# jdalcorso/radar-sounder-crw

Hardware: AMD Instinct MI355X
Metric: radargram columns/sec (CRW fwd+bwd) (higher is better)
Workload: dtype f32 (conv2-5 multiply on the bf16 matrix cores with hi/lo operand pairs, fp32 accumulate: fp32-grade; everything else fp32); 1 GPU; one synthetic 512x4096 radargram per GPU per step = 8 items [T=32,N=63,16x16] (patch 16x16, overlap (8, 0)), tau=0.01, CNN encoder, fwd+bwd+all-reduce+Adam; parallelism=dp1 (independent sequences), chain=fp32 MFMA 16x16x4, prefix form, encoder_convs=bf16x3

## Files before the change

### radar-sounder-crw_amd/csrc/encoder_front.hip

```cpp
#include "crw_common.h"
#include <type_traits>
#include <cstdlib>

namespace crw {
namespace {

typedef __bf16 bf8 __attribute__((ext_vector_type(8)));
typedef short s4v __attribute__((ext_vector_type(4)));
typedef short s8v __attribute__((ext_vector_type(8)));
typedef __attribute__((address_space(3))) char *lds_cp;

__device__ inline uint16_t f2bf(float x) { return __builtin_bit_cast(uint16_t, (__bf16)x); }
__device__ inline float bf2f(uint16_t h) { return __builtin_bit_cast(float, (uint32_t)h << 16); }

__device__ inline void lds_barrier() { asm volatile("s_waitcnt lgkmcnt(0)\n\ts_barrier" ::: "memory"); }

constexpr int XPW = 18;
constexpr int C1W = 14, C1N = C1W * C1W;
constexpr int A1W = 13, A1PW = 15;
constexpr int C2W = 11, C2N = C2W * C2W;
constexpr int OW = 10, ON = 100;
constexpr int D2PW = 19;
constexpr int D2HALF = D2PW * D2PW * 32;
constexpr int KS2 = 7;
// ... 271 lines not shown
    for (int e = tid; e < ON * 32; e += NT) {
      const int c = e & 31, q = e >> 5, y = q / OW, x = q % OW;
      if (oy0 + y < Ho && ox0 + x < Wo) {
        const float *s2 = L.c2r + (y * C2W + x) * 32 + c;
        const float v = fmaxf(fmaxf(s2[0], s2[32]), fmaxf(s2[C2W * 32], s2[C2W * 32 + 32]));
        const uint16_t h = f2bf(v);
        const long o = (((long)pt * Ho + oy0 + y) * Wo + ox0 + x) * 32 + c;
        a.f.yh[o] = h;
        if (SPLIT == 3) a.f.yl[o] = f2bf(v - bf2f(h));
      }
    }
  }
}

__global__ __launch_bounds__(256) void pack_w2_kernel(const float *__restrict__ w, uint16_t *fh, uint16_t *fl,
                                                      uint16_t *bh, uint16_t *bl) {
  for (int e = blockIdx.x * 256 + threadIdx.x; e < KS2 * 32 * 32; e += gridDim.x * 256) {
    const int k = e & 31, co = (e >> 5) & 31, s = e >> 10;
    const int tap = 4 * s + (k >> 3), ci = k & 7;
    const float v = tap < 25 ? w[(co * 8 + ci) * 25 + tap] : 0.f;
    const uint16_t h = f2bf(v);
    fh[e] = h;
    if (fl) fl[e] = f2bf(v - bf2f(h));
  }
  for (int e = blockIdx.x * 256 + threadIdx.x; e < 25 * 8 * 32; e += gridDim.x * 256) {
    const int co = e & 31, ci = (e >> 5) & 7, tap = e >> 8;
    const float v = w[(co * 8 + ci) * 25 + tap];
    const uint16_t h = f2bf(v);
    bh[e] = h;
    if (bl) bl[e] = f2bf(v - bf2f(h));
  }
}

struct FrontBwdArgs {
  FrontArgs f;
  const uint16_t *w2bh, *w2bl;
  const float *dy;
  float *part;
  int patches_per_block;
  long long *stamps;
  int H, W, tiles_x, tiles_y;
};
[[maybe_unused]] constexpr int NPHASE = 10;
#ifdef CRW_CONV_STAMPS
#define FRONT_STAMP(k)                                                       \
  if (a.stamps && tid == 0) {                                                \
    const long long now_ = (long long)__builtin_amdgcn_s_memtime();          \
    phase_[k] += now_ - prev_;                                               \
    prev_ = now_;                                                            \
  }
#else
#define FRONT_STAMP(k)
#endif

__device__ inline s4v tr_read0(uint32_t lds_addr) {
  s4v v;
  asm volatile("ds_read_b64_tr_b16 %0, %1" : "=v"(v) : "v"(lds_addr) : "memory");
  return v;
}
__device__ inline bf8 tr_pair(uint32_t a_lo, uint32_t a_hi) {
  const s4v lo = tr_read0(a_lo), hi = tr_read0(a_hi);
  const s8v v = {lo[0], lo[1], lo[2], lo[3], hi[0], hi[1], hi[2], hi[3]};
  return __builtin_bit_cast(bf8, v);
}

__device__ inline int argmax4(float a, float b, float c, float d) {
  int k = 0;
  float m = a;
  if (b > m) { m = b; k = 1; }
  if (c > m) { m = c; k = 2; }
  if (d > m) { m = d; k = 3; }
  return k;
}

template <int W, int CS>
__device__ inline float pool_bwd_pixel(const float *__restrict__ in, const float *__restrict__ dout, int y, int x, int c) {
  const float *ctr = in + ((y + 1) * (W + 2) + x + 1) * CS + c;
  float nb[3][3], dv[2][2];
#pragma unroll
  for (int dy = 0; dy < 3; ++dy)
#pragma unroll
    for (int dx = 0; dx < 3; ++dx) nb[dy][dx] = ctr[((dy - 1) * (W + 2) + (dx - 1)) * CS];
#pragma unroll
  for (int dyw = 0; dyw < 2; ++dyw)
#pragma unroll
    for (int dxw = 0; dxw < 2; ++dxw) {
      const int wy = min(max(y - dyw, 0), W - 2), wx = min(max(x - dxw, 0), W - 2);
      dv[dyw][dxw] = dout[(wy * (W - 1) + wx) * CS + c];
    }
  const float mine = nb[1][1];
  float gsum = 0.f;
#pragma unroll
  for (int dyw = 0; dyw < 2; ++dyw)
#pragma unroll
    for (int dxw = 0; dxw < 2; ++dxw) {
      const int wy = y - dyw, wx = x - dxw;
      bool win = mine > 0.f && wy >= 0 && wy < W - 1 && wx >= 0 && wx < W - 1;
      const int k = dyw * 2 + dxw;
#pragma unroll
      for (int j = 0; j < 4; ++j)
        if (j != k) {
          const float v = nb[1 - dyw + (j >> 1)][1 - dxw + (j & 1)];
          win = win && (j < k ? mine > v : mine >= v);
        }
      gsum += win ? dv[dyw][dxw] : 0.f;
    }
// ... 459 lines not shown
#pragma unroll
          for (int tx = 0; tx < 5; ++tx) {
            float s1 = 0.f;
#pragma unroll
            for (int x = 0; x < TCW / 2; ++x) s1 = fmaf(dv[x], xv[x + tx], s1);
            dw1[tx] += s1;
          }
        }
      }
    }
    lds_barrier();
  }

  const int PART = 32 * 8 * 25 + 32 + 8 * cin * 25 + 8;
  float *out = a.part + (long)blockIdx.x * PART;
#pragma unroll
  for (int uu = 0; uu < 2; ++uu) {
    const int tl = wave + NWV * uu;
    const int tap = 2 * (tl >> 1) + (r16 >> 3);
    if (tl < 26 && tap < 25)
#pragma unroll
      for (int r = 0; r < 4; ++r) out[((16 * (tl & 1) + 4 * g + r) * 8 + (r16 & 7)) * 25 + tap] = wacc[uu][r];
  }
  __syncthreads();
  float *red = reinterpret_cast<float *>(lds);
  red[tid] = db2;
  __syncthreads();
  if (tid < 32) {
    float s = 0.f;
    for (int k = 0; k < NTH / 32; ++k) s += red[tid + 32 * k];
    out[32 * 8 * 25 + tid] = s;
  }
  __syncthreads();
  if (tid < nrowthr)
#pragma unroll
    for (int tx = 0; tx < 5; ++tx) red[tid * 5 + tx] = dw1[tx];
  __syncthreads();
  if (tid < nout) {
    const int q = tid / 5, tx = tid % 5;
    float s = 0.f;
    for (int y = 0; y < nrp; ++y) s += red[(q * nrp + y) * 5 + tx];
    out[32 * 8 * 25 + 32 + tid] = s;
  }
  __syncthreads();
  red[tid] = db1;
  __syncthreads();
  if (tid < 8) {
    float s = 0.f;
    for (int k = 0; k < NTH / 8; ++k) s += red[tid + 8 * k];
    out[32 * 8 * 25 + 32 + nout + tid] = s;
  }
}

template <int SPLIT>
__global__ __launch_bounds__(NTH) void front_bwd_saved_kernel(FrontBwdArgs a) {
  extern __shared__ __attribute__((aligned(16))) char lds[];
  char *p = lds;
  const int cin = a.f.cin;
  auto take = [&](size_t bytes) { char *r = p; p += (bytes + 15) & ~(size_t)15; return r; };
  float *xs = (float *)take(sizeof(float) * cin * XPW * XPW);
  char *a1h = take(A1PW * A1PW * 16), *a1l = take(A1PW * A1PW * 16);
  char *wbh = take(25 * 8 * 32 * 2), *wbl = take(25 * 8 * 32 * 2);
  char *d2h = take(2 * D2HALF), *d2l = take(2 * D2HALF);
  float *dyb = (float *)take(sizeof(float) * ON * 32);
  char *k2s = take(SV_K2), *k1s = take(SV_K1);
  float *dA1 = dyb, *dC1 = dyb + A1W * A1W * 8;

  const int tid = threadIdx.x, lane = tid & 63, wave = tid >> 6, g = lane >> 4, r16 = lane & 15;
  for (int e = tid; e < cin * XPW * XPW; e += NTH) xs[e] = 0.f;
  for (int e = tid; e < A1PW * A1PW * 4; e += NTH) {
    reinterpret_cast<uint32_t *>(a1h)[e] = 0;
    reinterpret_cast<uint32_t *>(a1l)[e] = 0;
  }
  for (int e = tid; e < 25 * 8 * 32 / 8; e += NTH) {
    const int ch = e & 3, ci = (e >> 2) & 7, tap = e >> 5;
    const int d = ((tap * 2 + (ch >> 1)) * 8 + ci) * 2 + (ch & 1);
    reinterpret_cast<uint4 *>(wbh)[d] = reinterpret_cast<const uint4 *>(a.w2bh)[e];
    if (SPLIT == 3) reinterpret_cast<uint4 *>(wbl)[d] = reinterpret_cast<const uint4 *>(a.w2bl)[e];
  }
  for (int e = tid; e < 2 * D2HALF / 4; e += NTH) {
    reinterpret_cast<uint32_t *>(d2h)[e] = 0;
    reinterpret_cast<uint32_t *>(d2l)[e] = 0;
  }
  __syncthreads();

  f32x4 wacc[2];
  wacc[0] = f32x4{0.f, 0.f, 0.f, 0.f};
  wacc[1] = f32x4{0.f, 0.f, 0.f, 0.f};
  float db2 = 0.f, db1 = 0.f, dw1[5] = {0.f, 0.f, 0.f, 0.f, 0.f};
  const int nout = 8 * cin * 25, nrp = C1W / cin, nrowthr = 8 * cin * 5 * nrp;
  const uint32_t d2h_a = (uint32_t)(uintptr_t)(lds_cp)d2h, d2l_a = (uint32_t)(uintptr_t)(lds_cp)d2l;
  const uint32_t a1h_a = (uint32_t)(uintptr_t)(lds_cp)a1h, a1l_a = (uint32_t)(uintptr_t)(lds_cp)a1l;
  const int p_begin = blockIdx.x * a.patches_per_block;
  const int p_end = min(a.f.P, p_begin + a.patches_per_block);

  constexpr int NA1 = 2 * SV_A1 / 16, NK2 = SV_K2 / 16, NK1 = SV_K1 / 16, NSV = NA1 + NK2 + NK1;
  static_assert(NSV <= NTH && ON * 32 / 4 <= NTH, "one chunk per thread");
  typedef uint32_t u4v __attribute__((ext_vector_type(4)));
  float4 dy_r;
  float x_r = 0.f;
  u4v sv_r;
  const __amdgpu_buffer_rsrc_t dy_rs = __builtin_amdgcn_make_buffer_rsrc((void *)a.dy, 0, (int)((long)a.f.P * ON * 32 * 4), 0x00020000);
  const __amdgpu_buffer_rsrc_t x_rs = __builtin_amdgcn_make_buffer_rsrc((void *)a.f.x, 0, (int)((long)a.f.P * cin * 256 * 4), 0x00020000);
  const __amdgpu_buffer_rsrc_t sv_rs = __builtin_amdgcn_make_buffer_rsrc((void *)a.f.saved, 0, (int)((long)a.f.P * SV_BYTES), 0x00020000);
  auto fetch = [&](int pt) {
    dy_r = __builtin_bit_cast(float4, __builtin_amdgcn_raw_buffer_load_b128(dy_rs, tid * 16, pt * (ON * 32 * 4), 0));
    x_r = __builtin_bit_cast(float, __builtin_amdgcn_raw_buffer_load_b32(x_rs, tid * 4, pt * (cin * 256 * 4), 0));
    sv_r = __builtin_amdgcn_raw_buffer_load_b128(sv_rs, min(tid, NSV - 1) * 16, pt * SV_BYTES, 0);
  };
  if (p_begin < p_end) fetch(p_begin);
  for (int pt = p_begin; pt < p_end; ++pt) {
    if (tid < cin * 256) xs[((tid >> 8) * XPW + ((tid >> 4) & 15) + 1) * XPW + (tid & 15) + 1] = x_r;
    if (tid < ON * 32 / 4) reinterpret_cast<float4 *>(dyb)[tid] = dy_r;
    if (tid < NA1) {
      const int pl = tid / (A1W * A1W), px = tid % (A1W * A1W);
      *reinterpret_cast<u4v *>((pl ? a1l : a1h) + ((px / A1W + 1) * A1PW + px % A1W + 1) * 16) = sv_r;
    } else if (tid < NA1 + NK2) {
      reinterpret_cast<u4v *>(k2s)[tid - NA1] = sv_r;
    } else if (tid < NSV) {
      reinterpret_cast<u4v *>(k1s)[tid - NA1 - NK2] = sv_r;
    }
    if (pt + 1 < p_end) fetch(pt + 1);
    lds_barrier();

    for (int e = tid; e < C2N * 32; e += NTH) {
      const int co = e & 31, pix = e >> 5, y = pix / C2W, x = pix % C2W;
      float gsum = 0.f;
#pragma unroll
      for (int dyw = 0; dyw < 2; ++dyw)
#pragma unroll
        for (int dxw = 0; dxw < 2; ++dxw) {
          const int wy = y - dyw, wx = x - dxw;
          const bool ok = wy >= 0 && wy < OW && wx >= 0 && wx < OW;
          const int idx = (min(max(wy, 0), OW - 1) * OW + min(max(wx, 0), OW - 1)) * 32 + co;
          const int code = k2s[idx];
          const float d = dyb[idx];
          gsum += (ok && code == (4 | (dyw * 2 + dxw))) ? d : 0.f;
        }
      db2 += gsum;
      const uint16_t h = f2bf(gsum);
      const int o = (co >> 4) * D2HALF + ((y + 4) * D2PW + x + 4) * 32 + 2 * (co & 15);
      *reinterpret_cast<uint16_t *>(d2h + o) = h;
      if (SPLIT == 3) *reinterpret_cast<uint16_t *>(d2l + o) = f2bf(gsum - bf2f(h));
    }
    lds_barrier();

    {
      const int t16 = lane & 15, q = t16 >> 2, pq = t16 & 3;
#pragma unroll 1
      for (int ks = 0; ks < 4; ++ks) {
        const int i_lo = 32 * ks + 8 * g + q, i_hi = i_lo + 4;
        const bool v_lo = i_lo < C2N, v_hi = i_hi < C2N;
        const int y_lo = v_lo ? i_lo / C2W : 0, x_lo = v_lo ? i_lo % C2W : 0;
        const int y_hi = v_hi ? i_hi / C2W : 0, x_hi = v_hi ? i_hi % C2W : 0;
        const uint32_t ya_lo = (v_lo ? ((y_lo + 4) * D2PW + x_lo + 4) : 0) * 32 + 8 * (pq & 1) + 16 * (pq >> 1);
        const uint32_t ya_hi = (v_hi ? ((y_hi + 4) * D2PW + x_hi + 4) : 0) * 32 + 8 * (pq & 1) + 16 * (pq >> 1);
#pragma unroll
        for (int u = 0; u < 2; ++u) {
          const int tile = wave + NWV * u;
          if (tile < 26) {
            const int i = tile & 1, nt = tile >> 1;
            int tap = 2 * nt + (pq >> 1);
            if (tap > 24) tap = 24;
            const int toff = (tap / 5) * A1PW + (tap % 5);
            const uint32_t xa_lo = ((y_lo * A1PW + x_lo) + toff) * 16 + 8 * (pq & 1);
            const uint32_t xa_hi = ((y_hi * A1PW + x_hi) + toff) * 16 + 8 * (pq & 1);
            const bf8 ah = tr_pair(d2h_a + ya_lo + D2HALF * i, d2h_a + ya_hi + D2HALF * i);
            const bf8 bh = tr_pair(a1h_a + xa_lo, a1h_a + xa_hi);
            bf8 al, bl;
            if (SPLIT == 3) {
              al = tr_pair(d2l_a + ya_lo + D2HALF * i, d2l_a + ya_hi + D2HALF * i);
              bl = tr_pair(a1l_a + xa_lo, a1l_a + xa_hi);
            }
            asm volatile("s_waitcnt lgkmcnt(0)" ::: "memory");
            __builtin_amdgcn_sched_barrier(0);
            if (SPLIT == 3) {
              wacc[u] = __builtin_amdgcn_mfma_f32_16x16x32_bf16(al, bh, wacc[u], 0, 0, 0);
              wacc[u] = __builtin_amdgcn_mfma_f32_16x16x32_bf16(ah, bl, wacc[u], 0, 0, 0);
            }
            wacc[u] = __builtin_amdgcn_mfma_f32_16x16x32_bf16(ah, bh, wacc[u], 0, 0, 0);
          }
        }
      }
    }
    {
      f32x4 dacc = f32x4{0.f, 0.f, 0.f, 0.f}, dacc1 = dacc;
      if (wave < A1W) {
        const int xl = (r16 >= 4 && r16 < 12) ? r16 - 4 : (r16 < 4 ? 8 + r16 : 12);
        const int base = (wave + 5) * D2PW + xl + 5;
        const char *wb = ((SPLIT == 3 && r16 >= 8) ? wbl : wbh) + (g >> 1) * 256 + (r16 & 7) * 32 + (g & 1) * 16;
        const char *ab = d2h + (g >> 1) * D2HALF + (base - (4 * D2PW + 4)) * 32 + (g & 1) * 16;
        const long lo_a = d2l - d2h;
#pragma unroll
        for (int tap = 0; tap < 25; ++tap) {
          const int arel = ((4 - tap / 5) * D2PW + (4 - tap % 5)) * 32;
          const bf8 b = *reinterpret_cast<const bf8 *>(wb + tap * 512);
          const bf8 ah = *reinterpret_cast<const bf8 *>(ab + arel);
          if (SPLIT == 3) {
            const bf8 al = *reinterpret_cast<const bf8 *>(ab + lo_a + arel);
            dacc1 = __builtin_amdgcn_mfma_f32_16x16x32_bf16(al, b, dacc1, 0, 0, 0);
          }
          dacc = __builtin_amdgcn_mfma_f32_16x16x32_bf16(ah, b, dacc, 0, 0, 0);
        }
        if (SPLIT == 3) {
#pragma unroll
          for (int r = 0; r < 4; ++r) dacc[r] += __shfl_down(dacc[r], 8, 64) + dacc1[r];
        }
      }
      lds_barrier();
      if (wave < A1W && r16 < 8)
#pragma unroll
        for (int r = 0; r < 4; ++r) {
          const int row = 4 * g + r;
          const int x = (row >= 4 && row < 12) ? row - 4 : (row < 4 ? 8 + row : 12);
          if (row < 13) dA1[(wave * A1W + x) * 8 + r16] = dacc[r];
        }
    }
    lds_barrier();

    for (int e = tid; e < C1N * 8; e += NTH) {
      const int co = e & 7, pix = e >> 3, y = pix / C1W, x = pix % C1W;
      float gsum = 0.f;
#pragma unroll
      for (int dyw = 0; dyw < 2; ++dyw)
#pragma unroll
        for (int dxw = 0; dxw < 2; ++dxw) {
          const int wy = y - dyw, wx = x - dxw;
          const bool ok = wy >= 0 && wy < A1W && wx >= 0 && wx < A1W;
          const int idx = (min(max(wy, 0), A1W - 1) * A1W + min(max(wx, 0), A1W - 1)) * 8 + co;
          const int code = k1s[idx];
          const float d = dA1[idx];
          gsum += (ok && code == (4 | (dyw * 2 + dxw))) ? d : 0.f;
        }
      dC1[co * C1N + pix] = gsum;
      db1 += gsum;
    }
    lds_barrier();

    if (tid < nrowthr) {
      const int rp = tid % nrp, q = tid / nrp, ty = q % 5, ci = (q / 5) % cin, co = q / (5 * cin);
      for (int y = rp; y < C1W; y += nrp) {
        const float *dr = dC1 + co * C1N + y * C1W, *xr = xs + (ci * XPW + y + ty) * XPW;
        float dv[C1W], xv[XPW];
#pragma unroll
        for (int x = 0; x < C1W; ++x) dv[x] = dr[x];
#pragma unroll
        for (int x = 0; x < XPW; ++x) xv[x] = xr[x];
#pragma unroll
        for (int tx = 0; tx < 5; ++tx) {
          float s1 = 0.f;
#pragma unroll
          for (int x = 0; x < C1W; ++x) s1 = fmaf(dv[x], xv[x + tx], s1);
          dw1[tx] += s1;
        }
      }
    }
    lds_barrier();
  }

  const int PART = 32 * 8 * 25 + 32 + 8 * cin * 25 + 8;
  float *out = a.part + (long)blockIdx.x * PART;
#pragma unroll
  for (int u = 0; u < 2; ++u) {
    const int tile = wave + NWV * u;
    const int tap = 2 * (tile >> 1) + (r16 >> 3);
    if (tile < 26 && tap < 25)
#pragma unroll
      for (int r = 0; r < 4; ++r) out[((16 * (tile & 1) + 4 * g + r) * 8 + (r16 & 7)) * 25 + tap] = wacc[u][r];
  }
  __syncthreads();
  float *red = reinterpret_cast<float *>(lds);
  red[tid] = db2;
  __syncthreads();
  if (tid < 32) {
    float s = 0.f;
    for (int k = 0; k < NTH / 32; ++k) s += red[tid + 32 * k];
    out[32 * 8 * 25 + tid] = s;
  }
  __syncthreads();
  if (tid < nrowthr)
#pragma unroll
    for (int tx = 0; tx < 5; ++tx) red[tid * 5 + tx] = dw1[tx];
  __syncthreads();
  if (tid < nout) {
    const int q = tid / 5, tx = tid % 5;
    float s = 0.f;
    for (int y = 0; y < nrp; ++y) s += red[(q * nrp + y) * 5 + tx];
    out[32 * 8 * 25 + 32 + tid] = s;
  }
  __syncthreads();
  red[tid] = db1;
  __syncthreads();
  if (tid < 8) {
    float s = 0.f;
    for (int k = 0; k < NTH / 8; ++k) s += red[tid + 8 * k];
    out[32 * 8 * 25 + 32 + nout + tid] = s;
  }
}

struct FrontSums {
  const float *part;
  int nslice, stride, n;
  int end[4];
  float *dst[4];
};
__global__ __launch_bounds__(256) void front_slice_sum_kernel(FrontSums a) {
  const int e = blockIdx.x * 4 + (threadIdx.x >> 6), lane = threadIdx.x & 63;
  if (e >= a.n) return;
  float s = 0.f;
  for (int k = lane; k < a.nslice; k += 64) s += a.part[(long)k * a.stride + e];
  s = wave_sum(s);
  if (lane == 0) {
    const int seg = e < a.end[0] ? 0 : e < a.end[1] ? 1 : e < a.end[2] ? 2 : 3;
    a.dst[seg][e - (seg ? a.end[seg - 1] : 0)] = s;
  }
}

size_t fwd_lds_bytes(int cin, bool pad = false) {
  auto r = [](size_t b) { return (b + 15) & ~(size_t)15; };
  const size_t c1 = pad ? (C1W + 2) * (C1W + 2) : C1N, c2 = pad ? (C2W + 2) * (C2W + 2) : C2N;
  return r(4 * cin * XPW * XPW) + r(4 * (8 * cin * 25 + 8)) + r(4 * c1 * 8) + 2 * r(A1PW * A1PW * 16) +
         2 * r(KS2 * 32 * 32 * 2) + r(4 * c2 * 32);
}
size_t bwd_lds_bytes(int cin) {
  auto r = [](size_t b) { return (b + 15) & ~(size_t)15; };
  return fwd_lds_bytes(cin, true) + 2 * r(25 * 8 * 32 * 2) + 2 * r(2 * D2HALF) + r(4 * ON * 32);
}
size_t bwd_saved_lds_bytes(int cin) {
  auto r = [](size_t b) { return (b + 15) & ~(size_t)15; };
  return r(4 * cin * XPW * XPW) + 2 * r(A1PW * A1PW * 16) + 2 * r(25 * 8 * 32 * 2) + 2 * r(2 * D2HALF) + r(4 * ON * 32) + r(SV_K2) + r(SV_K1);
}
int front_slices(int P) { return P < 256 ? P : 256; }

}
}

using namespace crw;

long long *g_front_stamps = nullptr;

extern "C" {

#ifdef CRW_CONV_STAMPS
void crw_debug_front_stamps(long long *buf) { g_front_stamps = buf; }
#endif

int crw_enc_front_pack(const float *w2, uint16_t *fwd_hi, uint16_t *fwd_lo, uint16_t *bwd_hi, uint16_t *bwd_lo,
                       crw_stream_t stream) {
  clear_stale_error();
  if (!w2 || !fwd_hi || !bwd_hi || (fwd_lo == nullptr) != (bwd_lo == nullptr)) return CRW_EINVAL;
  hipLaunchKernelGGL(pack_w2_kernel, dim3(28), dim3(256), 0, (hipStream_t)stream, w2, fwd_hi, fwd_lo, bwd_hi, bwd_lo);
  return check_launch();
}

static int front_fwd_threads() {
  static const int nt = [] { const char *e = getenv("CRW_FRONT_NT"); return e && atoi(e) == 1024 ? 1024 : 512; }();
  return nt;
}

size_t crw_enc_front_saved_bytes(int P) { return P < 1 ? 0 : (size_t)P * SV_BYTES; }

int crw_enc_front_fwd(int split, const float *x, int P, int cin, const float *w1, const float *b1,
                      const uint16_t *w2_hi, const uint16_t *w2_lo, const float *b2, uint16_t *y_hi, uint16_t *y_lo,
                      void *saved, crw_stream_t stream) {
  clear_stale_error();
  if (!x || !w1 || !b1 || !w2_hi || !b2 || !y_hi || P < 1 || (cin != 1 && cin != 2) || (split != 1 && split != 3))
    return CRW_EINVAL;
  if (split == 3 && (!w2_lo || !y_lo)) return CRW_EINVAL;
  FrontArgs a{x, w1, b1, w2_hi, w2_lo, b2, y_hi, y_lo, P, cin, static_cast<char *>(saved)};
  const size_t lds = fwd_lds_bytes(cin);
  const int grid = P < 512 ? P : 512;
  if (front_fwd_threads() == 1024) {
    if (split == 3) hipLaunchKernelGGL((front_fwd_kernel<3, 1024>), dim3(grid), dim3(1024), lds, (hipStream_t)stream, a);
    else hipLaunchKernelGGL((front_fwd_kernel<1, 1024>), dim3(grid), dim3(1024), lds, (hipStream_t)stream, a);
  } else {
    if (split == 3) hipLaunchKernelGGL((front_fwd_kernel<3, 512>), dim3(grid), dim3(512), lds, (hipStream_t)stream, a);
    else hipLaunchKernelGGL((front_fwd_kernel<1, 512>), dim3(grid), dim3(512), lds, (hipStream_t)stream, a);
  }
  return check_launch();
}

int crw_enc_front_fwd_map(int split, const float *x, int P, int cin, int H, int W, const float *w1, const float *b1,
                          const uint16_t *w2_hi, const uint16_t *w2_lo, const float *b2, uint16_t *y_hi, uint16_t *y_lo,
                          crw_stream_t stream) {
  clear_stale_error();
  if (!x || !w1 || !b1 || !w2_hi || !b2 || !y_hi || P < 1 || (cin != 1 && cin != 2) || (split != 1 && split != 3) || H < 7 ||
      W < 7)
    return CRW_EINVAL;
  if (split == 3 && (!w2_lo || !y_lo)) return CRW_EINVAL;
  const int tx = (W - 6 + OW - 1) / OW, ty = (H - 6 + OW - 1) / OW;
  FrontMapArgs a{{x, w1, b1, w2_hi, w2_lo, b2, y_hi, y_lo, P, cin}, H, W, tx, ty};
  auto r = [](size_t b) { return (b + 15) & ~(size_t)15; };
  const size_t lds = r(4 * cin * MXW * MXW) + r(4 * (8 * cin * 25 + 8)) + r(4 * MC1W * MC1W * 8) + 2 * r(A1PW * A1PW * 16) +
                     2 * r(KS2 * 32 * 32 * 2) + r(4 * C2N * 32);
  const long nwork = (long)P * tx * ty;
  const int grid = nwork < 512 ? (int)nwork : 512;
  const bool big = front_fwd_threads() == 1024;
  static bool attr[4] = {false, false, false, false};
  const void *fns[4] = {(const void *)front_fwd_map_kernel<1, 512>, (const void *)front_fwd_map_kernel<3, 512>,
                        (const void *)front_fwd_map_kernel<1, 1024>, (const void *)front_fwd_map_kernel<3, 1024>};
  const int which = (big ? 2 : 0) + (split == 3 ? 1 : 0);
  if (!attr[which] && lds > 64 * 1024) {
    if (hipFuncSetAttribute(fns[which], hipFuncAttributeMaxDynamicSharedMemorySize, (int)lds) != hipSuccess) return CRW_EHIP;
    attr[which] = true;
  }
  if (big) {
    if (split == 3) hipLaunchKernelGGL((front_fwd_map_kernel<3, 1024>), dim3(grid), dim3(1024), lds, (hipStream_t)stream, a);
    else hipLaunchKernelGGL((front_fwd_map_kernel<1, 1024>), dim3(grid), dim3(1024), lds, (hipStream_t)stream, a);
  } else {
    if (split == 3) hipLaunchKernelGGL((front_fwd_map_kernel<3, 512>), dim3(grid), dim3(512), lds, (hipStream_t)stream, a);
    else hipLaunchKernelGGL((front_fwd_map_kernel<1, 512>), dim3(grid), dim3(512), lds, (hipStream_t)stream, a);
  }
  return check_launch();
}

size_t crw_enc_front_ws_bytes(int P, int cin) {
  if (P < 1 || (cin != 1 && cin != 2)) return 0;
  return (size_t)front_slices(P) * (32 * 8 * 25 + 32 + 8 * cin * 25 + 8) * sizeof(float);
}

int crw_enc_front_bwd(int split, const float *x, int P, int cin, const float *w1, const float *b1,
                      const uint16_t *w2_hi, const uint16_t *w2_lo, const float *b2, const uint16_t *w2b_hi,
                      const uint16_t *w2b_lo, const float *dy, const void *saved, float *dw1, float *db1, float *dw2, float *db2,
                      void *ws, size_t ws_bytes, crw_stream_t stream) {
  clear_stale_error();
  if (!x || !w1 || !b1 || !w2_hi || !b2 || !w2b_hi || !dy || !dw1 || !db1 || !dw2 || !db2 || !ws || P < 1 ||
      (cin != 1 && cin != 2) || (split != 1 && split != 3))
    return CRW_EINVAL;
  if (split == 3 && (!w2_lo || !w2b_lo)) return CRW_EINVAL;
  if (ws_bytes < crw_enc_front_ws_bytes(P, cin)) return CRW_EWORKSPACE;
  hipStream_t s = (hipStream_t)stream;
  const int nslice = front_slices(P), ppb = (P + nslice - 1) / nslice;
  FrontBwdArgs a{{x, w1, b1, w2_hi, w2_lo, b2, nullptr, nullptr, P, cin, const_cast<char *>(static_cast<const char *>(saved))},
                 w2b_hi, w2b_lo, dy, (float *)ws, ppb, g_front_stamps};
  static const char *force_rc = getenv("CRW_FRONT_RECOMPUTE");
  if (saved && !(force_rc && force_rc[0] == '1')) {
    const size_t ldss = bwd_saved_lds_bytes(cin);
    static bool sattr3 = false, sattr1 = false;
    bool &sattr = split == 3 ? sattr3 : sattr1;
    const void *fn = split == 3 ? (const void *)front_bwd_saved_kernel<3> : (const void *)front_bwd_saved_kernel<1>;
    if (!sattr) {
      if (hipFuncSetAttribute(fn, hipFuncAttributeMaxDynamicSharedMemorySize, 160 * 1024) != hipSuccess) return CRW_EHIP;
      sattr = true;
    }
    if (split == 3) hipLaunchKernelGGL(front_bwd_saved_kernel<3>, dim3(nslice), dim3(NTH), ldss, s, a);
    else hipLaunchKernelGGL(front_bwd_saved_kernel<1>, dim3(nslice), dim3(NTH), ldss, s, a);
    CRW_TRY(check_launch());
    const int n2 = 32 * 8 * 25, n1 = 8 * cin * 25, PART = n2 + 32 + n1 + 8;
    FrontSums fs{(float *)ws, nslice, PART, n2 + 32 + n1 + 8, {n2, n2 + 32, n2 + 32 + n1, n2 + 32 + n1 + 8}, {dw2, db2, dw1, db1}};
    hipLaunchKernelGGL(front_slice_sum_kernel, dim3((fs.n + 3) / 4), dim3(256), 0, s, fs);
    return check_launch();
  }
  const size_t lds = bwd_lds_bytes(cin);
  static bool attr3 = false, attr1 = false;
  if (split == 3) {
    if (!attr3) {
      if (hipFuncSetAttribute((const void *)front_bwd_kernel<3>, hipFuncAttributeMaxDynamicSharedMemorySize, 160 * 1024) !=
          hipSuccess) return CRW_EHIP;
      attr3 = true;
    }
    hipLaunchKernelGGL(front_bwd_kernel<3>, dim3(nslice), dim3(NTH), lds, s, a);
  } else {
    if (!attr1) {
      if (hipFuncSetAttribute((const void *)front_bwd_kernel<1>, hipFuncAttributeMaxDynamicSharedMemorySize, 160 * 1024) !=
          hipSuccess) return CRW_EHIP;
      attr1 = true;
    }
    hipLaunchKernelGGL(front_bwd_kernel<1>, dim3(nslice), dim3(NTH), lds, s, a);
  }
  CRW_TRY(check_launch());
  const int n2 = 32 * 8 * 25, n1 = 8 * cin * 25, PART = n2 + 32 + n1 + 8;
  float *part = (float *)ws;
  FrontSums fs{part, nslice, PART, n2 + 32 + n1 + 8, {n2, n2 + 32, n2 + 32 + n1, n2 + 32 + n1 + 8}, {dw2, db2, dw1, db1}};
  hipLaunchKernelGGL(front_slice_sum_kernel, dim3((fs.n + 3) / 4), dim3(256), 0, s, fs);
  return check_launch();
}


int crw_enc_front_bwd_map(int split, const float *x, int P, int cin, int H, int W, const float *w1, const float *b1,
                          const uint16_t *w2_hi, const uint16_t *w2_lo, const float *b2, const uint16_t *w2b_hi,
                          const uint16_t *w2b_lo, const float *dy, float *dw1, float *db1, float *dw2, float *db2, void *ws,
                          size_t ws_bytes, crw_stream_t stream) {
  clear_stale_error();
  if (!x || !w1 || !b1 || !w2_hi || !b2 || !w2b_hi || !dy || !dw1 || !db1 || !dw2 || !db2 || !ws || P < 1 ||
      (cin != 1 && cin != 2) || (split != 1 && split != 3) || H < 7 || W < 7)
    return CRW_EINVAL;
  if (split == 3 && (!w2_lo || !w2b_lo)) return CRW_EINVAL;
  const int tx = (W - 6 + OW - 1) / OW, ty = (H - 6 + OW - 1) / OW;
  const long units_l = (long)P * tx * ty;
  if (units_l > 0x7fffffffL) return CRW_EINVAL;
  const int units = (int)units_l;
  if (ws_bytes < crw_enc_front_ws_bytes(units, cin)) return CRW_EWORKSPACE;
  hipStream_t s = (hipStream_t)stream;
  int nslice = front_slices(units);
  const int upb = (units + nslice - 1) / nslice;
  nslice = (units + upb - 1) / upb;
  FrontBwdArgs a{{x, w1, b1, w2_hi, w2_lo, b2, nullptr, nullptr, P, cin, nullptr}, w2b_hi, w2b_lo, dy, (float *)ws, upb, nullptr, H, W, tx, ty};
  const void *fn = split == 3 ? (const void *)front_bwd_tile_kernel<3> : (const void *)front_bwd_tile_kernel<1>;
  static bool attr3 = false, attr1 = false;
// ... 20 lines not shown
```

Before: 643,900 radargram columns/s.

## Retune saved front backward kernel for two workgroups per CU with 512 threads

Templates the saved-activation encoder front backward kernel on thread count (default 512 instead of NTH), doubles the slice grid to 512, and shrinks the LDS footprint with a tighter dY2 padding layout. The aim is to fit two workgroups per CU and improve latency hiding. It also hoists the A-operand transposed loads out of the per-tile loop in the weight-gradient MFMA, splits the conv1 weight-gradient row loop into halves to cut register pressure, and adds phase timestamps. The costs are more per-thread work loops, more partial slices to reduce, and an extra LDS buffer for overflow dw1 rows.

```diff
diff --git a/radar-sounder-crw_amd/csrc/encoder_front.hip b/radar-sounder-crw_amd/csrc/encoder_front.hip
--- a/radar-sounder-crw_amd/csrc/encoder_front.hip
+++ b/radar-sounder-crw_amd/csrc/encoder_front.hip
@@ -347,6 +347,11 @@
 #else
 #define FRONT_STAMP(k)
 #endif
+
+__device__ inline int opaque(int v) {
+  asm volatile("" : "+v"(v));
+  return v;
+}
 
 __device__ inline s4v tr_read0(uint32_t lds_addr) {
   s4v v;
@@ -912,8 +917,23 @@
   }
 }
 
-template <int SPLIT>
-__global__ __launch_bounds__(NTH) void front_bwd_saved_kernel(FrontBwdArgs a) {
+constexpr int D2SW = C2W + 3;
+constexpr int D2SHALF = (C2W * D2SW + 3) * 32;
+constexpr int W1ROWS = 560;
+constexpr int W1X = W1ROWS - 512;
+
+template <int SPLIT, int NT>
+__global__ __launch_bounds__(NT) __attribute__((amdgpu_waves_per_eu(4))) void front_bwd_saved_kernel(FrontBwdArgs a) {
+#ifndef CRW_FRONT_FETCH_AT
+#define CRW_FRONT_FETCH_AT 0
+#endif
+  constexpr int FETCH_AT = CRW_FRONT_FETCH_AT;
+  constexpr int NW = NT / 64;
+  constexpr int VL = NTH / NT;
+  constexpr int VW = (W1ROWS + NT - 1) / NT;
+  constexpr int WU = (26 + NW - 1) / NW;
+  constexpr int RU = (A1W + NW - 1) / NW;
+  static_assert(NTH % NT == 0 && NW % 2 == 0 && 2 * 256 <= NT, "thread count");
   extern __shared__ __attribute__((aligned(16))) char lds[];
   char *p = lds;
   const int cin = a.f.cin;
@@ -921,208 +941,279 @@
   float *xs = (float *)take(sizeof(float) * cin * XPW * XPW);
   char *a1h = take(A1PW * A1PW * 16), *a1l = take(A1PW * A1PW * 16);
   char *wbh = take(25 * 8 * 32 * 2), *wbl = take(25 * 8 * 32 * 2);
-  char *d2h = take(2 * D2HALF), *d2l = take(2 * D2HALF);
+  char *d2h = take(2 * D2SHALF), *d2l = take(2 * D2SHALF);
   float *dyb = (float *)take(sizeof(float) * ON * 32);
   char *k2s = take(SV_K2), *k1s = take(SV_K1);
+  float *w1x = (float *)take(sizeof(float) * W1X * 5);
   float *dA1 = dyb, *dC1 = dyb + A1W * A1W * 8;
 
   const int tid = threadIdx.x, lane = tid & 63, wave = tid >> 6, g = lane >> 4, r16 = lane & 15;
-  for (int e = tid; e < cin * XPW * XPW; e += NTH) xs[e] = 0.f;
-  for (int e = tid; e < A1PW * A1PW * 4; e += NTH) {
+  for (int e = tid; e < W1X * 5; e += NT) w1x[e] = 0.f;
+  for (int e = tid; e < cin * XPW * XPW; e += NT) xs[e] = 0.f;
+  for (int e = tid; e < A1PW * A1PW * 4; e += NT) {
     reinterpret_cast<uint32_t *>(a1h)[e] = 0;
     reinterpret_cast<uint32_t *>(a1l)[e] = 0;
   }
-  for (int e = tid; e < 25 * 8 * 32 / 8; e += NTH) {
+  for (int e = tid; e < 25 * 8 * 32 / 8; e += NT) {
     const int ch = e & 3, ci = (e >> 2) & 7, tap = e >> 5;
     const int d = ((tap * 2 + (ch >> 1)) * 8 + ci) * 2 + (ch & 1);
     reinterpret_cast<uint4 *>(wbh)[d] = reinterpret_cast<const uint4 *>(a.w2bh)[e];
     if (SPLIT == 3) reinterpret_cast<uint4 *>(wbl)[d] = reinterpret_cast<const uint4 *>(a.w2bl)[e];
   }
-  for (int e = tid; e < 2 * D2HALF / 4; e += NTH) {
+  for (int e = tid; e < 2 * D2SHALF / 4; e += NT) {
     reinterpret_cast<uint32_t *>(d2h)[e] = 0;
     reinterpret_cast<uint32_t *>(d2l)[e] = 0;
   }
   __syncthreads();
 
-  f32x4 wacc[2];
-  wacc[0] = f32x4{0.f, 0.f, 0.f, 0.f};
-  wacc[1] = f32x4{0.f, 0.f, 0.f, 0.f};
-  float db2 = 0.f, db1 = 0.f, dw1[5] = {0.f, 0.f, 0.f, 0.f, 0.f};
+  f32x4 wacc[WU];
+#pragma unroll
+  for (int u = 0; u < WU; ++u) wacc[u] = f32x4{0.f, 0.f, 0.f, 0.f};
+  float db2[VL], db1[VL], dw1[5] = {0.f, 0.f, 0.f, 0.f, 0.f};
+#pragma unroll
+  for (int v = 0; v < VL; ++v) db2[v] = db1[v] = 0.f;
   const int nout = 8 * cin * 25, nrp = C1W / cin, nrowthr = 8 * cin * 5 * nrp;
   const uint32_t d2h_a = (uint32_t)(uintptr_t)(lds_cp)d2h, d2l_a = (uint32_t)(uintptr_t)(lds_cp)d2l;
   const uint32_t a1h_a = (uint32_t)(uintptr_t)(lds_cp)a1h, a1l_a = (uint32_t)(uintptr_t)(lds_cp)a1l;
   const int p_begin = blockIdx.x * a.patches_per_block;
   const int p_end = min(a.f.P, p_begin + a.patches_per_block);
-
-  constexpr int NA1 = 2 * SV_A1 / 16, NK2 = SV_K2 / 16, NK1 = SV_K1 / 16, NSV = NA1 + NK2 + NK1;
-  static_assert(NSV <= NTH && ON * 32 / 4 <= NTH, "one chunk per thread");
+#ifdef CRW_CONV_STAMPS
+  long long phase_[NPHASE] = {0, 0, 0, 0, 0, 0, 0, 0, 0, 0}, prev_ = (long long)__builtin_amdgcn_s_memtime();
+#endif
+
+  constexpr int NA1 = 2 * SV_A1 / 16, NK2 = SV_K2 / 16, NK1 = SV_K1 / 16, NSV = NA1 + NK2 + NK1, NDY = ON * 32 / 4;
+  constexpr int DYIT = (NDY + NT - 1) / NT, SVIT = (NSV + NT - 1) / NT;
   typedef uint32_t u4v __attribute__((ext_vector_type(4)));
-  float4 dy_r;
+  float4 dy_r[DYIT];
   float x_r = 0.f;
-  u4v sv_r;
+  u4v sv_r[SVIT];
   const __amdgpu_buffer_rsrc_t dy_rs = __builtin_amdgcn_make_buffer_rsrc((void *)a.dy, 0, (int)((long)a.f.P * ON * 32 * 4), 0x00020000);
   const __amdgpu_buffer_rsrc_t x_rs = __builtin_amdgcn_make_buffer_rsrc((void *)a.f.x, 0, (int)((long)a.f.P * cin * 256 * 4), 0x00020000);
   const __amdgpu_buffer_rsrc_t sv_rs = __builtin_amdgcn_make_buffer_rsrc((void *)a.f.saved, 0, (int)((long)a.f.P * SV_BYTES), 0x00020000);
   auto fetch = [&](int pt) {
-    dy_r = __builtin_bit_cast(float4, __builtin_amdgcn_raw_buffer_load_b128(dy_rs, tid * 16, pt * (ON * 32 * 4), 0));
+#pragma unroll
+    for (int i = 0; i < DYIT; ++i)
+      dy_r[i] = __builtin_bit_cast(float4, __builtin_amdgcn_raw_buffer_load_b128(dy_rs, min(tid + i * NT, NDY - 1) * 16, pt * (ON * 32 * 4), 0));
     x_r = __builtin_bit_cast(float, __builtin_amdgcn_raw_buffer_load_b32(x_rs, tid * 4, pt * (cin * 256 * 4), 0));
-    sv_r = __builtin_amdgcn_raw_buffer_load_b128(sv_rs, min(tid, NSV - 1) * 16, pt * SV_BYTES, 0);
+#pragma unroll
+    for (int i = 0; i < SVIT; ++i)
+      sv_r[i] = __builtin_amdgcn_raw_buffer_load_b128(sv_rs, min(tid + i * NT, NSV - 1) * 16, pt * SV_BYTES, 0);
   };
   if (p_begin < p_end) fetch(p_begin);
   for (int pt = p_begin; pt < p_end; ++pt) {
     if (tid < cin * 256) xs[((tid >> 8) * XPW + ((tid >> 4) & 15) + 1) * XPW + (tid & 15) + 1] = x_r;
-    if (tid < ON * 32 / 4) reinterpret_cast<float4 *>(dyb)[tid] = dy_r;
-    if (tid < NA1) {
-      const int pl = tid / (A1W * A1W), px = tid % (A1W * A1W);
-      *reinterpret_cast<u4v *>((pl ? a1l : a1h) + ((px / A1W + 1) * A1PW + px % A1W + 1) * 16) = sv_r;
-    } else if (tid < NA1 + NK2) {
-      reinterpret_cast<u4v *>(k2s)[tid - NA1] = sv_r;
-    } else if (tid < NSV) {
-      reinterpret_cast<u4v *>(k1s)[tid - NA1 - NK2] = sv_r;
-    }
-    if (pt + 1 < p_end) fetch(pt + 1);
-    lds_barrier();
-
-    for (int e = tid; e < C2N * 32; e += NTH) {
-      const int co = e & 31, pix = e >> 5, y = pix / C2W, x = pix % C2W;
-      float gsum = 0.f;
-#pragma unroll
-      for (int dyw = 0; dyw < 2; ++dyw)
-#pragma unroll
-        for (int dxw = 0; dxw < 2; ++dxw) {
-          const int wy = y - dyw, wx = x - dxw;
-          const bool ok = wy >= 0 && wy < OW && wx >= 0 && wx < OW;
-          const int idx = (min(max(wy, 0), OW - 1) * OW + min(max(wx, 0), OW - 1)) * 32 + co;
-          const int code = k2s[idx];
-          const float d = dyb[idx];
-          gsum += (ok && code == (4 | (dyw * 2 + dxw))) ? d : 0.f;
-        }
-      db2 += gsum;
-      const uint16_t h = f2bf(gsum);
-      const int o = (co >> 4) * D2HALF + ((y + 4) * D2PW + x + 4) * 32 + 2 * (co & 15);
-      *reinterpret_cast<uint16_t *>(d2h + o) = h;
-      if (SPLIT == 3) *reinterpret_cast<uint16_t *>(d2l + o) = f2bf(gsum - bf2f(h));
-    }
-    lds_barrier();
+#pragma unroll
+    for (int i = 0; i < DYIT; ++i)
+      if (tid + i * NT < NDY) reinterpret_cast<float4 *>(dyb)[tid + i * NT] = dy_r[i];
+#pragma unroll
+    for (int i = 0; i < SVIT; ++i) {
+      const int c = opaque(tid) + i * NT;
+      if (c < NA1) {
+        const int pl = c / (A1W * A1W), px = c % (A1W * A1W);
+        *reinterpret_cast<u4v *>((pl ? a1l : a1h) + ((px / A1W + 1) * A1PW + px % A1W + 1) * 16) = sv_r[i];
+      } else if (c < NA1 + NK2) {
+        reinterpret_cast<u4v *>(k2s)[c - NA1] = sv_r[i];
+      } else if (c < NSV) {
+        reinterpret_cast<u4v *>(k1s)[c - NA1 - NK2] = sv_r[i];
+      }
+    }
+    if (FETCH_AT == 0 && pt + 1 < p_end) fetch(pt + 1);
+    lds_barrier();
+    FRONT_STAMP(0)
+
+    for (int e0 = opaque(tid); e0 < C2N * 32; e0 += NTH) {
+#pragma unroll
+      for (int v = 0; v < VL; ++v) {
+        const int e = e0 + NT * v;
+        if (e < C2N * 32) {
+          const int co = e & 31, pix = e >> 5, y = pix / C2W, x = pix % C2W;
+          float gsum = 0.f;
+#pragma unroll
+          for (int dyw = 0; dyw < 2; ++dyw)
+#pragma unroll
+            for (int dxw = 0; dxw < 2; ++dxw) {
+              const int wy = y - dyw, wx = x - dxw;
+              const bool ok = wy >= 0 && wy < OW && wx >= 0 && wx < OW;
+              const int idx = (min(max(wy, 0), OW - 1) * OW + min(max(wx, 0), OW - 1)) * 32 + co;
+              const int code = k2s[idx];
+              const float d = dyb[idx];
+              gsum += (ok && code == (4 | (dyw * 2 + dxw))) ? d : 0.f;
+            }
+          db2[v] += gsum;
+          const uint16_t h = f2bf(gsum);
+          const int o = (co >> 4) * D2SHALF + (y * D2SW + x + 3) * 32 + 2 * (co & 15);
+          *reinterpret_cast<uint16_t *>(d2h + o) = h;
+          if (SPLIT == 3) *reinterpret_cast<uint16_t *>(d2l + o) = f2bf(gsum - bf2f(h));
+        }
+      }
+    }
+    lds_barrier();
+    FRONT_STAMP(4)
 
     {
-      const int t16 = lane & 15, q = t16 >> 2, pq = t16 & 3;
+      const int ln = opaque(lane), t16 = ln & 15, q = t16 >> 2, pq = t16 & 3, ih = wave & 1;
 #pragma unroll 1
       for (int ks = 0; ks < 4; ++ks) {
-        const int i_lo = 32 * ks + 8 * g + q, i_hi = i_lo + 4;
+        const int i_lo = 32 * ks + 8 * (ln >> 4) + q, i_hi = i_lo + 4;
         const bool v_lo = i_lo < C2N, v_hi = i_hi < C2N;
         const int y_lo = v_lo ? i_lo / C2W : 0, x_lo = v_lo ? i_lo % C2W : 0;
         const int y_hi = v_hi ? i_hi / C2W : 0, x_hi = v_hi ? i_hi % C2W : 0;
-        const uint32_t ya_lo = (v_lo ? ((y_lo + 4) * D2PW + x_lo + 4) : 0) * 32 + 8 * (pq & 1) + 16 * (pq >> 1);
-        const uint32_t ya_hi = (v_hi ? ((y_hi + 4) * D2PW + x_hi + 4) : 0) * 32 + 8 * (pq & 1) + 16 * (pq >> 1);
-#pragma unroll
-        for (int u = 0; u < 2; ++u) {
-          const int tile = wave + NWV * u;
+        const uint32_t ya_lo = (v_lo ? y_lo * D2SW + x_lo + 3 : 0) * 32 + 8 * (pq & 1) + 16 * (pq >> 1) + D2SHALF * ih;
+        const uint32_t ya_hi = (v_hi ? y_hi * D2SW + x_hi + 3 : 0) * 32 + 8 * (pq & 1) + 16 * (pq >> 1) + D2SHALF * ih;
+        const bf8 ah = tr_pair(d2h_a + ya_lo, d2h_a + ya_hi);
+        bf8 al, bh[WU], bl[WU];
+        if (SPLIT == 3) al = tr_pair(d2l_a + ya_lo, d2l_a + ya_hi);
+#pragma unroll
+        for (int u = 0; u < WU; ++u) {
+          const int tile = wave + NW * u;
           if (tile < 26) {
-            const int i = tile & 1, nt = tile >> 1;
-            int tap = 2 * nt + (pq >> 1);
+            int tap = 2 * (tile >> 1) + (pq >> 1);
             if (tap > 24) tap = 24;
             const int toff = (tap / 5) * A1PW + (tap % 5);
             const uint32_t xa_lo = ((y_lo * A1PW + x_lo) + toff) * 16 + 8 * (pq & 1);
             const uint32_t xa_hi = ((y_hi * A1PW + x_hi) + toff) * 16 + 8 * (pq & 1);
-            const bf8 ah = tr_pair(d2h_a + ya_lo + D2HALF * i, d2h_a + ya_hi + D2HALF * i);
-            const bf8 bh = tr_pair(a1h_a + xa_lo, a1h_a + xa_hi);
-            bf8 al, bl;
+            bh[u] = tr_pair(a1h_a + xa_lo, a1h_a + xa_hi);
+            if (SPLIT == 3) bl[u] = tr_pair(a1l_a + xa_lo, a1l_a + xa_hi);
+          }
+        }
+        asm volatile("s_waitcnt lgkmcnt(0)" ::: "memory");
+        __builtin_amdgcn_sched_barrier(0);
+#pragma unroll
+        for (int u = 0; u < WU; ++u) {
+          if (wave + NW * u < 26) {
             if (SPLIT == 3) {
-              al = tr_pair(d2l_a + ya_lo + D2HALF * i, d2l_a + ya_hi + D2HALF * i);
-              bl = tr_pair(a1l_a + xa_lo, a1l_a + xa_hi);
+              wacc[u] = __builtin_amdgcn_mfma_f32_16x16x32_bf16(al, bh[u], wacc[u], 0, 0, 0);
+              wacc[u] = __builtin_amdgcn_mfma_f32_16x16x32_bf16(ah, bl[u], wacc[u], 0, 0, 0);
             }
-            asm volatile("s_waitcnt lgkmcnt(0)" ::: "memory");
+            wacc[u] = __builtin_amdgcn_mfma_f32_16x16x32_bf16(ah, bh[u], wacc[u], 0, 0, 0);
+          }
+        }
+      }
+    }
+    FRONT_STAMP(5)
+    {
+      f32x4 dacc[RU], dacc1[RU];
+      const int ln = opaque(lane), g = ln >> 4, r16 = ln & 15;
+      const int xl = (r16 >= 4 && r16 < 12) ? r16 - 4 : (r16 < 4 ? 8 + r16 : 12);
+      const char *wb = ((SPLIT == 3 && r16 >= 8) ? wbl : wbh) + (g >> 1) * 256 + (r16 & 7) * 32 + (g & 1) * 16;
+      const char *ab = d2h + (g >> 1) * D2SHALF + (g & 1) * 16 + (xl - 3 * D2SW) * 32;
+      const long lo_a = d2l - d2h;
+#pragma unroll
+      for (int u = 0; u < RU; ++u) {
+        dacc[u] = f32x4{0.f, 0.f, 0.f, 0.f};
+        dacc1[u] = dacc[u];
+        const int row = wave + NW * u;
+        const char *abr = ab + row * (D2SW * 32);
+        if (row < A1W) {
+#pragma unroll
+          for (int ty = 0; ty < 5; ++ty) {
+            const int y = row + 1 - ty;
+            if (y >= 0 && y < C2W) {
+#pragma unroll
+              for (int tx = 0; tx < 5; ++tx) {
+                const int arel = ((4 - ty) * D2SW + (4 - tx)) * 32;
+                const bf8 b = *reinterpret_cast<const bf8 *>(wb + (ty * 5 + tx) * 512);
+                const bf8 ah = *reinterpret_cast<const bf8 *>(abr + arel);
+                if (SPLIT == 3) {
+                  const bf8 al = *reinterpret_cast<const bf8 *>(abr + lo_a + arel);
+                  dacc1[u] = __builtin_amdgcn_mfma_f32_16x16x32_bf16(al, b, dacc1[u], 0, 0, 0);
+                }
+                dacc[u] = __builtin_amdgcn_mfma_f32_16x16x32_bf16(ah, b, dacc[u], 0, 0, 0);
+              }
+            }
+          }
+          if (SPLIT == 3) {
+#pragma unroll
+            for (int r = 0; r < 4; ++r) dacc[u][r] += __shfl_down(dacc[u][r], 8, 64) + dacc1[u][r];
+          }
+        }
+      }
+      lds_barrier();
+#pragma unroll
+      for (int u = 0; u < RU; ++u) {
+        const int row = wave + NW * u;
+        if (row < A1W && r16 < 8)
+#pragma unroll
+          for (int r = 0; r < 4; ++r) {
+            const int trow = 4 * g + r;
+            const int x = (trow >= 4 && trow < 12) ? trow - 4 : (trow < 4 ? 8 + trow : 12);
+            if (trow < 13) dA1[(row * A1W + x) * 8 + r16] = dacc[u][r];
+          }
+      }
+    }
+    lds_barrier();
+    FRONT_STAMP(6)
+    if (FETCH_AT == 1 && pt + 1 < p_end) fetch(pt + 1);
+
+    for (int e0 = opaque(tid); e0 < C1N * 8; e0 += NTH) {
+#pragma unroll
+      for (int v = 0; v < VL; ++v) {
+        const int e = e0 + NT * v;
+        if (e < C1N * 8) {
+          const int co = e & 7, pix = e >> 3, y = pix / C1W, x = pix % C1W;
+          float gsum = 0.f;
+#pragma unroll
+          for (int dyw = 0; dyw < 2; ++dyw)
+#pragma unroll
+            for (int dxw = 0; dxw < 2; ++dxw) {
+              const int wy = y - dyw, wx = x - dxw;
+              const bool ok = wy >= 0 && wy < A1W && wx >= 0 && wx < A1W;
+              const int idx = (min(max(wy, 0), A1W - 1) * A1W + min(max(wx, 0), A1W - 1)) * 8 + co;
+              const int code = k1s[idx];
+              const float d = dA1[idx];
+              gsum += (ok && code == (4 | (dyw * 2 + dxw))) ? d : 0.f;
+            }
+          dC1[co * C1N + pix] = gsum;
+          db1[v] += gsum;
+        }
+      }
+    }
+    lds_barrier();
+    FRONT_STAMP(7)
+    if (FETCH_AT == 2 && pt + 1 < p_end) fetch(pt + 1);
+
+#pragma unroll
+    for (int v = 0; v < VW; ++v) {
+      const int it = opaque(tid) + NT * v;
+      if (it < nrowthr) {
+        const int rp = it % nrp, q = it / nrp, ty = q % 5, ci = (q / 5) % cin, co = q / (5 * cin);
+        for (int y = rp; y < C1W; y += nrp) {
+          const float *dr = dC1 + co * C1N + y * C1W, *xr = xs + (ci * XPW + y + ty) * XPW;
+          float s1[5] = {0.f, 0.f, 0.f, 0.f, 0.f};
+#pragma unroll
+          for (int h = 0; h < 2; ++h) {
+            float xv[C1W / 2 + 4], dv[C1W / 2];
+#pragma unroll
+            for (int x = 0; x < C1W / 2 + 4; ++x) xv[x] = xr[h * (C1W / 2) + x];
+#pragma unroll
+            for (int x = 0; x < C1W / 2; ++x) dv[x] = dr[h * (C1W / 2) + x];
+#pragma unroll
+            for (int x = 0; x < C1W / 2; ++x)
+#pragma unroll
+              for (int tx = 0; tx < 5; ++tx) s1[tx] = fmaf(dv[x], xv[x + tx], s1[tx]);
             __builtin_amdgcn_sched_barrier(0);
-            if (SPLIT == 3) {
-              wacc[u] = __builtin_amdgcn_mfma_f32_16x16x32_bf16(al, bh, wacc[u], 0, 0, 0);
-              wacc[u] = __builtin_amdgcn_mfma_f32_16x16x32_bf16(ah, bl, wacc[u], 0, 0, 0);
-            }
-            wacc[u] = __builtin_amdgcn_mfma_f32_16x16x32_bf16(ah, bh, wacc[u], 0, 0, 0);
           }
-        }
-      }
-    }
-    {
-      f32x4 dacc = f32x4{0.f, 0.f, 0.f, 0.f}, dacc1 = dacc;
-      if (wave < A1W) {
-        const int xl = (r16 >= 4 && r16 < 12) ? r16 - 4 : (r16 < 4 ? 8 + r16 : 12);
-        const int base = (wave + 5) * D2PW + xl + 5;
-        const char *wb = ((SPLIT == 3 && r16 >= 8) ? wbl : wbh) + (g >> 1) * 256 + (r16 & 7) * 32 + (g & 1) * 16;
-        const char *ab = d2h + (g >> 1) * D2HALF + (base - (4 * D2PW + 4)) * 32 + (g & 1) * 16;
-        const long lo_a = d2l - d2h;
-#pragma unroll
-        for (int tap = 0; tap < 25; ++tap) {
-          const int arel = ((4 - tap / 5) * D2PW + (4 - tap % 5)) * 32;
-          const bf8 b = *reinterpret_cast<const bf8 *>(wb + tap * 512);
-          const bf8 ah = *reinterpret_cast<const bf8 *>(ab + arel);
-          if (SPLIT == 3) {
-            const bf8 al = *reinterpret_cast<const bf8 *>(ab + lo_a + arel);
-            dacc1 = __builtin_amdgcn_mfma_f32_16x16x32_bf16(al, b, dacc1, 0, 0, 0);
+#pragma unroll
+          for (int tx = 0; tx < 5; ++tx) {
+            if (v == 0) dw1[tx] += s1[tx];
+            else w1x[(it - NT) * 5 + tx] += s1[tx];
           }
-          dacc = __builtin_amdgcn_mfma_f32_16x16x32_bf16(ah, b, dacc, 0, 0, 0);
-        }
-        if (SPLIT == 3) {
-#pragma unroll
-          for (int r = 0; r < 4; ++r) dacc[r] += __shfl_down(dacc[r], 8, 64) + dacc1[r];
-        }
-      }
-      lds_barrier();
-      if (wave < A1W && r16 < 8)
-#pragma unroll
-        for (int r = 0; r < 4; ++r) {
-          const int row = 4 * g + r;
-          const int x = (row >= 4 && row < 12) ? row - 4 : (row < 4 ? 8 + row : 12);
-          if (row < 13) dA1[(wave * A1W + x) * 8 + r16] = dacc[r];
-        }
-    }
-    lds_barrier();
-
-    for (int e = tid; e < C1N * 8; e += NTH) {
-      const int co = e & 7, pix = e >> 3, y = pix / C1W, x = pix % C1W;
-      float gsum = 0.f;
-#pragma unroll
-      for (int dyw = 0; dyw < 2; ++dyw)
-#pragma unroll
-        for (int dxw = 0; dxw < 2; ++dxw) {
-          const int wy = y - dyw, wx = x - dxw;
-          const bool ok = wy >= 0 && wy < A1W && wx >= 0 && wx < A1W;
-          const int idx = (min(max(wy, 0), A1W - 1) * A1W + min(max(wx, 0), A1W - 1)) * 8 + co;
-          const int code = k1s[idx];
-          const float d = dA1[idx];
-          gsum += (ok && code == (4 | (dyw * 2 + dxw))) ? d : 0.f;
-        }
-      dC1[co * C1N + pix] = gsum;
-      db1 += gsum;
-    }
-    lds_barrier();
-
-    if (tid < nrowthr) {
-      const int rp = tid % nrp, q = tid / nrp, ty = q % 5, ci = (q / 5) % cin, co = q / (5 * cin);
-      for (int y = rp; y < C1W; y += nrp) {
-        const float *dr = dC1 + co * C1N + y * C1W, *xr = xs + (ci * XPW + y + ty) * XPW;
-        float dv[C1W], xv[XPW];
-#pragma unroll
-        for (int x = 0; x < C1W; ++x) dv[x] = dr[x];
-#pragma unroll
-        for (int x = 0; x < XPW; ++x) xv[x] = xr[x];
-#pragma unroll
-        for (int tx = 0; tx < 5; ++tx) {
-          float s1 = 0.f;
-#pragma unroll
-          for (int x = 0; x < C1W; ++x) s1 = fmaf(dv[x], xv[x + tx], s1);
-          dw1[tx] += s1;
-        }
-      }
-    }
-    lds_barrier();
-  }
+        }
+      }
+    }
+    lds_barrier();
+    FRONT_STAMP(8)
+  }
+#ifdef CRW_CONV_STAMPS
+  if (a.stamps && tid == 0)
+    for (int k = 0; k < NPHASE; ++k) a.stamps[(long)blockIdx.x * NPHASE + k] = phase_[k];
+#endif
 
   const int PART = 32 * 8 * 25 + 32 + 8 * cin * 25 + 8;
   float *out = a.part + (long)blockIdx.x * PART;
 #pragma unroll
-  for (int u = 0; u < 2; ++u) {
-    const int tile = wave + NWV * u;
+  for (int u = 0; u < WU; ++u) {
+    const int tile = wave + NW * u;
     const int tap = 2 * (tile >> 1) + (r16 >> 3);
     if (tile < 26 && tap < 25)
 #pragma unroll
@@ -1130,7 +1221,8 @@
   }
   __syncthreads();
   float *red = reinterpret_cast<float *>(lds);
-  red[tid] = db2;
+#pragma unroll
+  for (int v = 0; v < VL; ++v) red[tid + NT * v] = db2[v];
   __syncthreads();
   if (tid < 32) {
     float s = 0.f;
@@ -1138,9 +1230,16 @@
     out[32 * 8 * 25 + tid] = s;
   }
   __syncthreads();
+  float w1x_r[5];
+#pragma unroll
+  for (int tx = 0; tx < 5; ++tx) w1x_r[tx] = (VW > 1 && tid < W1X) ? w1x[tid * 5 + tx] : 0.f;
+  __syncthreads();
   if (tid < nrowthr)
 #pragma unroll
     for (int tx = 0; tx < 5; ++tx) red[tid * 5 + tx] = dw1[tx];
+  if (VW > 1 && tid < W1X)
+#pragma unroll
+    for (int tx = 0; tx < 5; ++tx) red[(tid + NT) * 5 + tx] = w1x_r[tx];
   __syncthreads();
   if (tid < nout) {
     const int q = tid / 5, tx = tid % 5;
@@ -1149,7 +1248,8 @@
     out[32 * 8 * 25 + 32 + tid] = s;
   }
   __syncthreads();
-  red[tid] = db1;
+#pragma unroll
+  for (int v = 0; v < VL; ++v) red[tid + NT * v] = db1[v];
   __syncthreads();
   if (tid < 8) {
     float s = 0.f;
@@ -1188,9 +1288,12 @@
 }
 size_t bwd_saved_lds_bytes(int cin) {
   auto r = [](size_t b) { return (b + 15) & ~(size_t)15; };
-  return r(4 * cin * XPW * XPW) + 2 * r(A1PW * A1PW * 16) + 2 * r(25 * 8 * 32 * 2) + 2 * r(2 * D2HALF) + r(4 * ON * 32) + r(SV_K2) + r(SV_K1);
-}
+  return r(4 * cin * XPW * XPW) + 2 * r(A1PW * A1PW * 16) + 2 * r(25 * 8 * 32 * 2) + 2 * r(2 * D2SHALF) + r(4 * ON * 32) + r(SV_K2) + r(SV_K1) + r(4 * W1X * 5);
+}
+static_assert(4 * 2 * XPW * XPW + 2 * A1PW * A1PW * 16 + 2 * 25 * 8 * 32 * 2 + 4 * D2SHALF + 4 * ON * 32 + SV_K2 + SV_K1 + 4 * W1X * 5 + 64 <= 80 * 1024,
+              "front_bwd_saved_kernel: two workgroups per CU");
 int front_slices(int P) { return P < 256 ? P : 256; }
+int front_pair_slices(int P) { return P < 512 ? P : 512; }
 
 }
 }
@@ -1213,7 +1316,7 @@
   return check_launch();
 }
 
-static int front_fwd_threads() {
+static int front_threads() {
   static const int nt = [] { const char *e = getenv("CRW_FRONT_NT"); return e && atoi(e) == 1024 ? 1024 : 512; }();
   return nt;
 }
@@ -1230,7 +1333,7 @@
   FrontArgs a{x, w1, b1, w2_hi, w2_lo, b2, y_hi, y_lo, P, cin, static_cast<char *>(saved)};
   const size_t lds = fwd_lds_bytes(cin);
   const int grid = P < 512 ? P : 512;
-  if (front_fwd_threads() == 1024) {
+  if (front_threads() == 1024) {
     if (split == 3) hipLaunchKernelGGL((front_fwd_kernel<3, 1024>), dim3(grid), dim3(1024), lds, (hipStream_t)stream, a);
     else hipLaunchKernelGGL((front_fwd_kernel<1, 1024>), dim3(grid), dim3(1024), lds, (hipStream_t)stream, a);
   } else {
@@ -1255,7 +1358,7 @@
                      2 * r(KS2 * 32 * 32 * 2) + r(4 * C2N * 32);
   const long nwork = (long)P * tx * ty;
   const int grid = nwork < 512 ? (int)nwork : 512;
-  const bool big = front_fwd_threads() == 1024;
+  const bool big = front_threads() == 1024;
   static bool attr[4] = {false, false, false, false};
   const void *fns[4] = {(const void *)front_fwd_map_kernel<1, 512>, (const void *)front_fwd_map_kernel<3, 512>,
                         (const void *)front_fwd_map_kernel<1, 1024>, (const void *)front_fwd_map_kernel<3, 1024>};
@@ -1276,7 +1379,7 @@
 
 size_t crw_enc_front_ws_bytes(int P, int cin) {
   if (P < 1 || (cin != 1 && cin != 2)) return 0;
-  return (size_t)front_slices(P) * (32 * 8 * 25 + 32 + 8 * cin * 25 + 8) * sizeof(float);
+  return (size_t)front_pair_slices(P) * (32 * 8 * 25 + 32 + 8 * cin * 25 + 8) * sizeof(float);
 }
 
 int crw_enc_front_bwd(int split, const float *x, int P, int cin, const float *w1, const float *b1,
@@ -1290,21 +1393,28 @@
   if (split == 3 && (!w2_lo || !w2b_lo)) return CRW_EINVAL;
   if (ws_bytes < crw_enc_front_ws_bytes(P, cin)) return CRW_EWORKSPACE;
   hipStream_t s = (hipStream_t)stream;
-  const int nslice = front_slices(P), ppb = (P + nslice - 1) / nslice;
+  const int nslice = front_pair_slices(P), ppb = (P + nslice - 1) / nslice;
   FrontBwdArgs a{{x, w1, b1, w2_hi, w2_lo, b2, nullptr, nullptr, P, cin, const_cast<char *>(static_cast<const char *>(saved))},
                  w2b_hi, w2b_lo, dy, (float *)ws, ppb, g_front_stamps};
   static const char *force_rc = getenv("CRW_FRONT_RECOMPUTE");
   if (saved && !(force_rc && force_rc[0] == '1')) {
     const size_t ldss = bwd_saved_lds_bytes(cin);
-    static bool sattr3 = false, sattr1 = false;
-    bool &sattr = split == 3 ? sattr3 : sattr1;
-    const void *fn = split == 3 ? (const void *)front_bwd_saved_kernel<3> : (const void *)front_bwd_saved_kernel<1>;
-    if (!sattr) {
-      if (hipFuncSetAttribute(fn, hipFuncAttributeMaxDynamicSharedMemorySize, 160 * 1024) != hipSuccess) return CRW_EHIP;
-      sattr = true;
-    }
-    if (split == 3) hipLaunchKernelGGL(front_bwd_saved_kernel<3>, dim3(nslice), dim3(NTH), ldss, s, a);
-    else hipLaunchKernelGGL(front_bwd_saved_kernel<1>, dim3(nslice), dim3(NTH), ldss, s, a);
+    const bool big = front_threads() == 1024;
+    static bool sattr[4] = {false, false, false, false};
+    const void *fns[4] = {(const void *)front_bwd_saved_kernel<1, 512>, (const void *)front_bwd_saved_kernel<3, 512>,
+                          (const void *)front_bwd_saved_kernel<1, 1024>, (const void *)front_bwd_saved_kernel<3, 1024>};
+    const int which = (big ? 2 : 0) + (split == 3 ? 1 : 0);
+    if (!sattr[which]) {
+      if (hipFuncSetAttribute(fns[which], hipFuncAttributeMaxDynamicSharedMemorySize, (int)ldss) != hipSuccess) return CRW_EHIP;
+      sattr[which] = true;
+    }
+    if (big) {
+      if (split == 3) hipLaunchKernelGGL((front_bwd_saved_kernel<3, 1024>), dim3(nslice), dim3(1024), ldss, s, a);
+      else hipLaunchKernelGGL((front_bwd_saved_kernel<1, 1024>), dim3(nslice), dim3(1024), ldss, s, a);
+    } else {
+      if (split == 3) hipLaunchKernelGGL((front_bwd_saved_kernel<3, 512>), dim3(nslice), dim3(512), ldss, s, a);
+      else hipLaunchKernelGGL((front_bwd_saved_kernel<1, 512>), dim3(nslice), dim3(512), ldss, s, a);
+    }
     CRW_TRY(check_launch());
     const int n2 = 32 * 8 * 25, n1 = 8 * cin * 25, PART = n2 + 32 + n1 + 8;
     FrontSums fs{(float *)ws, nslice, PART, n2 + 32 + n1 + 8, {n2, n2 + 32, n2 + 32 + n1, n2 + 32 + n1 + 8}, {dw2, db2, dw1, db1}};
```

Result: no change. 649,000 radargram columns/s, median of 6 (+0.8%).
